# Farama-Foundation/Gymnasium-Robotics

Hardware: NVIDIA H100
Metric: env-steps/s (higher is better)
Workload: dtype f32

## Files before the change

### gymnasium_robotics_b200/csrc/sim_core.cuh

```cuda
#pragma once
#include "dmodel.h"

#if defined(__CUDACC__) || defined(B200_HOST_WARP)
#define B200_WARP_CODE 1
#endif
#ifdef __CUDACC__
#define HD static __device__ __forceinline__
#define HDN static __device__ __noinline__
#define STAGE static __device__ __noinline__
#define ASSUME_SHARED_PTR(p) __builtin_assume(__isShared(p))
#define ASSUME_SHARED(c) do { __builtin_assume(__isShared((c).s)); __builtin_assume(__isShared((c).mw)); __builtin_assume(__isShared((c).h)); } while (0)
#define WARP_W 32
#define SYNC() __syncwarp()
#define ALIGN() __syncthreads()
#define ALIGN_OR(p) __syncthreads_or(p)
#elif defined(B200_HOST_WARP)
#define HD static inline
#define HDN static
#define STAGE static
#define ASSUME_SHARED(c) do { } while (0)
#define ASSUME_SHARED_PTR(p) do { } while (0)
#define WARP_W 32
#define SYNC() __syncwarp()
#define ALIGN() __syncwarp()
// ... 1221 lines not shown
        else if (t2 == B200_GEOM_SPHERE) collide_plane_sphere(c, g1, g2, margin, o);
        else collide_plane_capsule(c, g1, g2, margin, o);
      } else if (t1 == B200_GEOM_BOX) collide_box_box(c, g1, g2, margin, o, bs);
      else if (t2 == B200_GEOM_BOX) collide_round_box(c, g1, g2, margin, o);
      else if (HF) collide_round_round(c, g1, g2, margin, o);
      float inc = margin - GF(pair_gap)[p];
      int k2 = 0;
      for (int k = 0; k < o.cnt; k++) if (o.dist[k] < inc) { if (k2 != k) { o.dist[k2] = o.dist[k]; for (int a = 0; a < 3; a++) { o.pos[k2][a] = o.pos[k][a]; o.nrm[k2][a] = o.nrm[k][a]; } } k2++; }
      o.cnt = k2;
    }
    int ocnt = o.cnt;
    int gtotal, gslot = wexscan(ocnt > 0 ? 1 : 0, c.lane, &gtotal);
    int basec = cnt[CNT_NCON], baseg = cnt[CNT_NGRP];
    int gid = baseg + gslot;
    if (ocnt > 0 && gid >= h->ngrp_max - DM_NWELD_MAX) ocnt = 0;
    int total, slot = wexscan(ocnt, c.lane, &total);
    SYNC();
    int kept = 0;
    for (int k = 0; k < ocnt; k++) {
      int id = basec + slot + k;
      if (id >= h->ncon_max) break;
      float* cr = SF(con) + id * CON_WORDS;
      cr[0] = o.pos[k][0]; cr[1] = o.pos[k][1]; cr[2] = o.pos[k][2];
      cr[3] = o.nrm[k][0]; cr[4] = o.nrm[k][1]; cr[5] = o.nrm[k][2];
      cr[6] = o.dist[k];
      ((int*)cr)[7] = p;
      ((int*)cr)[C_DIMGRP] = gid << 8;
      kept++;
    }
    if (ocnt > 0) {
      int* gi = (int*)(SF(group) + gid * GRP_WORDS);
      int ba = MI(geom_body)[PAIR_I(pair_geom1)[p]], bb = PAIR_I(pair_geom2)[p] < 0 ? 0 : MI(geom_body)[PAIR_I(pair_geom2)[p]];
      dmask_t ma = DM(body_ancdof, ba), mb = DM(body_ancdof, bb);
      const int bodies = GI(geom_mjb)[PAIR_I(pair_geom1)[p]] | ((PAIR_I(pair_geom2)[p] < 0 ? 0 : GI(geom_mjb)[PAIR_I(pair_geom2)[p]]) << 8);
      ((uint32_t*)gi)[G_RANGE] = (uint32_t)(basec + slot) | (uint32_t)kept << 8 | (uint32_t)bodies << 16;
      grp_set_masks(gi, ma ^ mb, mb);
    }
    if (c.lane == 0) {
      int nn = basec + total; if (nn > h->ncon_max) { nn = h->ncon_max; cnt[CNT_OVERFLOW] |= 2; }
      int ng = baseg + gtotal; if (ng > h->ngrp_max - DM_NWELD_MAX) { ng = h->ngrp_max - DM_NWELD_MAX; cnt[CNT_OVERFLOW] |= 4; }
      cnt[CNT_NCON] = nn; cnt[CNT_NGRP] = ng;
    }
    SYNC();
  }
  LANES(id, cnt[CNT_NCON]) {
    float* cr = SF(con) + id * CON_WORDS;
    const float pos[3] = {cr[0], cr[1], cr[2]}, dist = cr[6];
    float fr9[9] = {cr[3], cr[4], cr[5], 0, 0, 0, 0, 0, 0};
    const int p = ((const int*)cr)[7], gid8 = ((const int*)cr)[C_DIMGRP];
    make_frame(fr9);
    float r[3] = {pos[0] - h->ref[0], pos[1] - h->ref[1], pos[2] - h->ref[2]};
    for (int a = 0; a < 3; a++) { float* w = cr + C_W + 6 * a; cross3(w, r, fr9 + 3 * a); w[3] = fr9[3 * a]; w[4] = fr9[3 * a + 1]; w[5] = fr9[3 * a + 2]; }
    const float* fr = GF(pair_friction) + 3 * p;
    int dim = GI(pair_condim)[p];
    float mu0 = fr[0];
    cr[C_MU] = mu0; cr[C_MU + 1] = fr[1];
#ifdef B200_KITCHEN
    cr[C_MU + 2] = fr[2];
#endif
    float incl = PAIR_F(pair_margin)[p] - GF(pair_gap)[p];
    float solimp[5] = {GF(pair_solimp)[5 * p], GF(pair_solimp)[5 * p + 1], GF(pair_solimp)[5 * p + 2], GF(pair_solimp)[5 * p + 3], GF(pair_solimp)[5 * p + 4]};
    float solref[2] = {GF(pair_solref)[2 * p], GF(pair_solref)[2 * p + 1]};
    float imp = impedance(solimp, dist, incl);
    float K, Bc;
    ref_kb(c, solref, solimp[1], &K, &Bc);
    float tran = GF(pair_invweight)[2 * p];
    float R;
    if (dim == 1) R = fmaxf((1 - imp) / imp * tran, B200_MINVAL);
    else {
      float R0 = fmaxf((1 - imp) / imp * (tran + mu0 * mu0 * tran), B200_MINVAL);
      float mu = mu0 * rsqrtf(h->impratio);
      R = fmaxf(2 * mu * mu * R0, B200_MINVAL);
    }
    cr[C_D] = 1.0f / R;
    cr[C_U] = K * imp * (dist - incl); cr[C_U + 1] = 0; cr[C_U + 2] = 0; cr[C_U + 3] = 0;
#ifdef B200_KITCHEN
    cr[C_U + 4] = 0; cr[C_U + 5] = 0;
#endif
    cr[C_JV] = Bc;
    ((int*)cr)[C_DIMGRP] = dim | gid8;
    if (HF && h->nsensor > 0) {
      float* cx = SF(conx) + id * CX_WORDS;
      cx[CX_POS] = pos[0]; cx[CX_POS + 1] = pos[1]; cx[CX_POS + 2] = pos[2];
      ((int*)cx)[CX_PAIR] = p;
    }
  }
  SYNC();
}

#ifdef B200_KITCHEN
HD void con_w(const float* cr, int k, float* w) {
  if (k < 3) { const float* s = cr + C_W + 6 * k; w[0] = s[0]; w[1] = s[1]; w[2] = s[2]; w[3] = s[3]; w[4] = s[4]; w[5] = s[5]; }
  else { const float* s = cr + C_W + 6 * (k - 3) + 3; w[0] = s[0]; w[1] = s[1]; w[2] = s[2]; w[3] = w[4] = w[5] = 0; }
}
HD float con_mu(const float* cr, int k) { return k < 3 ? cr[C_MU] : (k == 3 ? cr[C_MU + 1] : cr[C_MU + 2]); }
#else
HD void con_w(const float* cr, int k, float* w) {
  if (k < 3) { const float* s = cr + C_W + 6 * k; w[0] = s[0]; w[1] = s[1]; w[2] = s[2]; w[3] = s[3]; w[4] = s[4]; w[5] = s[5]; }
  else { w[0] = cr[C_W + 3]; w[1] = cr[C_W + 4]; w[2] = cr[C_W + 5]; w[3] = w[4] = w[5] = 0; }
}
HD float con_mu(const float* cr, int k) { return k < 3 ? cr[C_MU] : cr[C_MU + 1]; }
#endif
HD int con_dim(const float* cr) { return ((const int*)cr)[C_DIMGRP] & 0xff; }
HD int con_grp(const float* cr) { return (((const int*)cr)[C_DIMGRP] >> 8) & 0xff; }
HD uint32_t con_act(const float* cr) { return ((const uint32_t*)cr)[C_DIMGRP] >> 16; }

template <bool HF>
STAGE void make_constraint(const Ctx c) {
  ASSUME_SHARED(c);
  const DMHead* h = c.h;
  int* cnt = SI(counters);
  if (c.lane == 0) { cnt[CNT_NDR] = 0; cnt[CNT_NWELD] = 0; }
  SYNC();
  for (int e = 0; e < h->neq; e++) {
    if (!MI(eq_active)[e] || MI(eq_type)[e] != B200_EQ_WELD) continue;
    const int nw = cnt[CNT_NWELD], gid = cnt[CNT_NGRP];
    float* wr = SF(weld) + nw * WELD_WORDS;
    const float* data = MF(eq_data) + 11 * e;
    int s1 = MI(eq_obj1)[e], s2 = MI(eq_obj2)[e], b1 = 0, b2 = 0;
    float p1[3] = {0, 0, 0}, p2[3] = {0, 0, 0}, q1[4] = {1, 0, 0, 0}, q2[4] = {1, 0, 0, 0}, t[3];
    if (s1 >= 0) { b1 = MI(site_body)[s1]; qmul(q1, SF(xquat) + 4 * b1, MF(site_quat) + 4 * s1); qrot(t, SF(xquat) + 4 * b1, MF(site_pos) + 3 * s1); for (int k = 0; k < 3; k++) p1[k] = SF(xpos)[3 * b1 + k] + t[k]; }
    if (s2 >= 0) { b2 = MI(site_body)[s2]; qmul(q2, SF(xquat) + 4 * b2, MF(site_quat) + 4 * s2); qrot(t, SF(xquat) + 4 * b2, MF(site_pos) + 3 * s2); for (int k = 0; k < 3; k++) p2[k] = SF(xpos)[3 * b2 + k] + t[k]; }
    qrot(t, q1, data + 3); for (int k = 0; k < 3; k++) p1[k] += t[k];
    qrot(t, q2, data + 0); for (int k = 0; k < 3; k++) p2[k] += t[k];
    const float ts = data[10];
    float quat[4], quat1[4] = {q2[0], -q2[1], -q2[2], -q2[3]}, quat2[4];
    qmul(quat, q1, data + 6);
    qmul(quat2, quat1, quat);
    const bool use1 = b1 > 0 && DM(body_ancdof, b1) != 0;
    float r[3];
    for (int k = 0; k < 3; k++) r[k] = (use1 ? p1[k] : p2[k]) - h->ref[k];
    float K, Bc;
    ref_kb(c, MF(eq_solref) + 2 * e, MF(eq_solimp)[5 * e + 1], &K, &Bc);
    LANES(k, 6) {
      float* w = wr + W_W + 6 * k;
      float cp;
      if (k < 3) {
        float e3[3] = {k == 0 ? 1.f : 0.f, k == 1 ? 1.f : 0.f, k == 2 ? 1.f : 0.f};
        cross3(w, r, e3); w[3] = e3[0]; w[4] = e3[1]; w[5] = e3[2];
        cp = k == 0 ? p1[0] - p2[0] : (k == 1 ? p1[1] - p2[1] : p1[2] - p2[2]);
      } else {
        const int kk = k - 3;
        for (int a = 0; a < 3; a++) {
          float qa[4] = {0, a == 0 ? 1.f : 0.f, a == 1 ? 1.f : 0.f, a == 2 ? 1.f : 0.f}, t1[4], t2[4];
          qmul(t1, quat1, qa); qmul(t2, t1, quat);
          w[a] = 0.5f * ts * (kk == 0 ? t2[1] : (kk == 1 ? t2[2] : t2[3])); w[3 + a] = 0;
        }
        cp = ts * (kk == 0 ? quat2[1] : (kk == 1 ? quat2[2] : quat2[3]));
      }
      float imp = impedance(MF(eq_solimp) + 5 * e, cp, 0.f);
      float R = fmaxf((1 - imp) / imp * MF(eq_invweight)[2 * e + (k < 3 ? 0 : 1)], B200_MINVAL);
      wr[W_D + k] = 1.0f / R; wr[W_JAR + k] = K * imp * cp;
    }
    if (c.lane == 0) {
      wr[W_B] = Bc;
      ((int*)wr)[W_GRP] = gid;
      int* gi = (int*)(SF(group) + gid * GRP_WORDS);
      dmask_t ma = DM(body_ancdof, b2), mb = DM(body_ancdof, b1);
      gi[G_RANGE] = 0;
      grp_set_masks(gi, ma ^ mb, mb);
    }
    SYNC();
    if (c.lane == 0) { cnt[CNT_NGRP] = gid + 1; cnt[CNT_NWELD] = nw + 1; }
    SYNC();
  }
  for (int base = 0; base < h->njnt; base += WARP_W) {
    int j = base + c.lane;
    int nrow = 0; float dist0 = 0, dist1 = 0, sgn0 = 0, sgn1 = 0;
    if (j < h->njnt && MI(jnt_limited)[j] && MI(jnt_type)[j] != B200_JNT_FREE) {
      float q = SF(qpos)[MI(jnt_qposadr)[j]], margin = MF(jnt_margin)[j];
      float dl = q - MF(jnt_range)[2 * j], du = MF(jnt_range)[2 * j + 1] - q;
      if (dl < margin) { dist0 = dl; sgn0 = 1.f; nrow = 1; }
      if (du < margin) { if (nrow) { dist1 = du; sgn1 = -1.f; } else { dist0 = du; sgn0 = -1.f; } nrow++; }
    }
    int total, slot = wexscan(nrow, c.lane, &total);
    int basec = cnt[CNT_NDR];
    SYNC();
#pragma unroll
    for (int k = 0; k < 2; k++) {
      int id = basec + slot + k;
      if (k >= nrow || id >= h->ndr_max) continue;
      const float distk = k ? dist1 : dist0, sgnk = k ? sgn1 : sgn0;
      float* dr = SF(dofrow) + id * DR_WORDS;
      int* di = (int*)dr;
      int d = MI(jnt_dofadr)[j];
      float margin = MF(jnt_margin)[j];
      float solimp[5] = {GF(jnt_solimp)[5 * j], GF(jnt_solimp)[5 * j + 1], GF(jnt_solimp)[5 * j + 2], GF(jnt_solimp)[5 * j + 3], GF(jnt_solimp)[5 * j + 4]};
      float solref[2] = {GF(jnt_solref)[2 * j], GF(jnt_solref)[2 * j + 1]};
      float imp = impedance(solimp, distk, margin);
      float K, Bc;
      ref_kb(c, solref, solimp[1], &K, &Bc);
      float R = fmaxf((1 - imp) / imp * MF(dof_invweight0)[d], B200_MINVAL);
      di[DR_DOF] = d; dr[DR_COEF] = sgnk; di[DR_DOF2] = -1; dr[DR_COEF2] = 0;
      dr[DR_D] = 1.0f / R; dr[DR_JAR] = K * imp * (distk - margin); dr[DR_JV] = Bc;
    }
    if (c.lane == 0) { int nn = basec + total; if (nn > h->ndr_max) { nn = h->ndr_max; cnt[CNT_OVERFLOW] |= 8; } cnt[CNT_NDR] = nn; }
    SYNC();
  }
  if (HF) for (int base = 0; base < h->nten; base += WARP_W) {
    int t = base + c.lane;
    int nrow = 0; float dist0 = 0, dist1 = 0, sgn0 = 0, sgn1 = 0;
    if (t < h->nten) {
      float len = MF(ten_coef)[2 * t] * SF(qpos)[MI(ten_qadr)[2 * t]];
      if (MI(ten_dof)[2 * t + 1] >= 0) len += MF(ten_coef)[2 * t + 1] * SF(qpos)[MI(ten_qadr)[2 * t + 1]];
      float margin = MF(ten_margin)[t];
      float dl = len - MF(ten_range)[2 * t], du = MF(ten_range)[2 * t + 1] - len;
      if (dl < margin) { dist0 = dl; sgn0 = 1.f; nrow = 1; }
      if (du < margin) { if (nrow) { dist1 = du; sgn1 = -1.f; } else { dist0 = du; sgn0 = -1.f; } nrow++; }
    }
    int total, slot = wexscan(nrow, c.lane, &total);
    int basec = cnt[CNT_NDR];
    SYNC();
#pragma unroll
    for (int k = 0; k < 2; k++) {
      int id = basec + slot + k;
      if (k >= nrow || id >= h->ndr_max) continue;
      const float distk = k ? dist1 : dist0, sgnk = k ? sgn1 : sgn0;
      float* dr = SF(dofrow) + id * DR_WORDS;
      int* di = (int*)dr;
      float margin = MF(ten_margin)[t];
      float solimp[5] = {GF(ten_solimp)[5 * t], GF(ten_solimp)[5 * t + 1], GF(ten_solimp)[5 * t + 2], GF(ten_solimp)[5 * t + 3], GF(ten_solimp)[5 * t + 4]};
      float solref[2] = {GF(ten_solref)[2 * t], GF(ten_solref)[2 * t + 1]};
      float imp = impedance(solimp, distk, margin);
      float K, Bc;
      ref_kb(c, solref, solimp[1], &K, &Bc);
      float R = fmaxf((1 - imp) / imp * GF(ten_invweight)[t], B200_MINVAL);
      di[DR_DOF] = MI(ten_dof)[2 * t]; dr[DR_COEF] = sgnk * MF(ten_coef)[2 * t];
      di[DR_DOF2] = MI(ten_dof)[2 * t + 1]; dr[DR_COEF2] = sgnk * MF(ten_coef)[2 * t + 1];
      dr[DR_D] = 1.0f / R; dr[DR_JAR] = K * imp * (distk - margin); dr[DR_JV] = Bc;
    }
    if (c.lane == 0) { int nn = basec + total; if (nn > h->ndr_max) { nn = h->ndr_max; cnt[CNT_OVERFLOW] |= 8; } cnt[CNT_NDR] = nn; }
    SYNC();
  }
#ifdef B200_KITCHEN
  if (c.lane == 0) {
    for (int e = 0; e < h->neq; e++) {
      if (!MI(eq_active)[e] || MI(eq_type)[e] != B200_EQ_JOINT) continue;
      int id = cnt[CNT_NDR];
      if (id >= h->ndr_max) { cnt[CNT_OVERFLOW] |= 8; break; }
      const float* data = MF(eq_data) + 11 * e;
      int j1 = MI(eq_obj1)[e], j2 = MI(eq_obj2)[e];
      float pos = SF(qpos)[MI(jnt_qposadr)[j1]] - MF(jnt_qpos0)[j1], deriv = 0.f;
      if (j2 >= 0) {
        float dif = SF(qpos)[MI(jnt_qposadr)[j2]] - MF(jnt_qpos0)[j2];
        pos -= data[0] + dif * (data[1] + dif * (data[2] + dif * (data[3] + dif * data[4])));
        deriv = data[1] + dif * (2 * data[2] + dif * (3 * data[3] + dif * 4 * data[4]));
      } else pos -= data[0];
      float* dr = SF(dofrow) + id * DR_WORDS;
      int* di = (int*)dr;
      float imp = impedance(MF(eq_solimp) + 5 * e, pos, 0.f);
      float K, Bc;
      ref_kb(c, MF(eq_solref) + 2 * e, MF(eq_solimp)[5 * e + 1], &K, &Bc);
      float R = fmaxf((1 - imp) / imp * MF(eq_invweight)[2 * e], B200_MINVAL);
      di[DR_DOF] = MI(jnt_dofadr)[j1]; dr[DR_COEF] = 1.f;
      di[DR_DOF2] = j2 >= 0 ? MI(jnt_dofadr)[j2] : -1; dr[DR_COEF2] = -deriv;
      dr[DR_D] = -1.0f / R; dr[DR_JAR] = K * imp * pos; dr[DR_JV] = Bc;
      cnt[CNT_NDR] = id + 1;
    }
  }
  SYNC();
#endif
  if (HF) { LANES(d, h->nfric) SF(fric)[d] = 0.f; SYNC(); }
}

HD uint32_t contact_base_forces(const float* cr, int dim, const float (&U)[C_NB], float* F) {
  float D = cr[C_D], un = U[0];
#pragma unroll
  for (int k = 0; k < C_NB; k++) F[k] = 0;
  if (dim == 1) { F[0] = un < 0 ? -D * un : 0.f; return un < 0 ? 1u : 0u; }
  uint32_t act = 0;
#pragma unroll
  for (int k = 1; k < C_NB; k++) {
    if (k >= dim) continue;
    float mu = con_mu(cr, k), uk = U[k];
    float xp = un + mu * uk, xm = un - mu * uk;
    float fp = xp < 0 ? -D * xp : 0.f, fm = xm < 0 ? -D * xm : 0.f;
    act |= (xp < 0 ? 1u : 0u) << (2 * k - 2) | (xm < 0 ? 1u : 0u) << (2 * k - 1);
    F[0] += fp + fm;
    F[k] = mu * (fp - fm);
  }
  return act;
}
HD void contact_base_forces(const float* cr, int dim, float* F) {
  float U[C_NB];
#pragma unroll
  for (int k = 0; k < C_NB; k++) U[k] = cr[C_U + k];
  contact_base_forces(cr, dim, U, F);
}
HD void contact_park_forces(float* cr, const float (&U)[C_NB]) {
  int* dg = (int*)cr + C_DIMGRP;
  float F[C_NB];
  const uint32_t act = contact_base_forces(cr, *dg & 0xff, U, F);
#pragma unroll
  for (int k = 0; k < C_NB; k++) cr[C_JV + k] = F[k];
  *dg = (int)(((uint32_t)*dg & 0xffffu) | act << 16);
}

template <bool HF>
STAGE void rows_from_vec(const Ctx c, const float* vec) {
  ASSUME_SHARED(c);
  ASSUME_SHARED_PTR(vec);
  const int* cnt = SI(counters);
  int ngrp = cnt[CNT_NGRP];
  LANES(idx, ngrp * 6) {
    int g = idx / 6, a = idx - 6 * g;
    float* gr = SF(group) + g * GRP_WORDS;
    dmask_t S = grp_mask(gr), sg = grp_sign(gr);
    float acc = 0;
    while (S) { int j = ffs_pop(S); float t = SF(cdof)[6 * j + a] * vec[j]; acc += DBIT(sg, j) ? t : -t; }
    gr[G_V + a] = acc;
  }
  SYNC();
  LANES(i, cnt[CNT_NCON]) {
    float* cr = SF(con) + i * CON_WORDS;
    int dim = con_dim(cr), nbase = dim == 1 ? 1 : dim;
    const float* dV = SF(group) + con_grp(cr) * GRP_WORDS + G_V;
    for (int k = 0; k < nbase; k++) {
      float w[6];
      con_w(cr, k, w);
      cr[C_JV + k] = dot6(w, dV);
    }
  }
  LANES(i, cnt[CNT_NWELD] * 6) {
    float* wr = SF(weld) + (i / 6) * WELD_WORDS;
    int k = i % 6;
    const float* dV = SF(group) + ((const int*)wr)[W_GRP] * GRP_WORDS + G_V;
    wr[W_JV + k] = dot6(wr + W_W + 6 * k, dV);
  }
  LANES(i, cnt[CNT_NDR]) {
    float* dr = SF(dofrow) + i * DR_WORDS;
    const int* di = (const int*)dr;
    float val = dr[DR_COEF] * vec[di[DR_DOF]];
    if (di[DR_DOF2] >= 0) val += dr[DR_COEF2] * vec[di[DR_DOF2]];
    dr[DR_JV] = val;
  }
  if (HF) LANES(d, c.h->nfric) SF(fric)[c.h->nfric + d] = vec[d];
  SYNC();
}

template <bool HF>
STAGE void rows_begin(const Ctx c, const float* qvel, const float* qacc) {
  ASSUME_SHARED(c);
  ASSUME_SHARED_PTR(qvel); ASSUME_SHARED_PTR(qacc);
  const int* cnt = SI(counters);
  int ngrp = cnt[CNT_NGRP];
  float* dA = SF(H);
  LANES(idx, ngrp * 6) {
    int g = idx / 6, a = idx - 6 * g;
    float* gr = SF(group) + g * GRP_WORDS;
    dmask_t S = grp_mask(gr), sg = grp_sign(gr);
    float acc = 0, acc2 = 0;
    while (S) {
      int j = ffs_pop(S);
      float cd = SF(cdof)[6 * j + a], t = cd * qvel[j], t2 = cd * qacc[j];
      bool pos = DBIT(sg, j);
      acc += pos ? t : -t; acc2 += pos ? t2 : -t2;
    }
    gr[G_V + a] = acc; dA[idx] = acc2;
  }
  SYNC();
  LANES(i, cnt[CNT_NCON]) {
    float* cr = SF(con) + i * CON_WORDS;
    int dim = con_dim(cr), nbase = dim == 1 ? 1 : dim;
    const float* gr = SF(group) + con_grp(cr) * GRP_WORDS;
    const float* gA = dA + 6 * con_grp(cr);
    float Bc = cr[C_JV];
    float U[C_NB];
#pragma unroll
    for (int k = 0; k < C_NB; k++) {
      U[k] = 0.f;
      if (k >= nbase) continue;
      float w[6];
      con_w(cr, k, w);
      float u = cr[C_U + k];
      u += Bc * dot6(w, gr + G_V);
      u += dot6(w, gA);
      cr[C_U + k] = u;
      U[k] = u;
    }
    contact_park_forces(cr, U);
  }
  LANES(i, cnt[CNT_NWELD] * 6) {
    float* wr = SF(weld) + (i / 6) * WELD_WORDS;
    int k = i % 6;
    const int g = ((const int*)wr)[W_GRP];
    const float* gr = SF(group) + g * GRP_WORDS;
    float u = wr[W_JAR + k];
    u += wr[W_B] * dot6(wr + W_W + 6 * k, gr + G_V);
    u += dot6(wr + W_W + 6 * k, dA + 6 * g);
    wr[W_JAR + k] = u;
  }
  LANES(i, cnt[CNT_NDR]) {
    float* dr = SF(dofrow) + i * DR_WORDS;
    const int* di = (const int*)dr;
    float v1 = dr[DR_COEF] * qvel[di[DR_DOF]], v2 = dr[DR_COEF] * qacc[di[DR_DOF]];
    if (di[DR_DOF2] >= 0) { v1 += dr[DR_COEF2] * qvel[di[DR_DOF2]]; v2 += dr[DR_COEF2] * qacc[di[DR_DOF2]]; }
    float u = dr[DR_JAR];
    u += dr[DR_JV] * v1;
    u += v2;
    dr[DR_JAR] = u;
  }
  if (HF) LANES(d, c.h->nfric) {
    float* fr = SF(fric);
    float u = fr[d];
    u += MF(dof_fricB)[d] * qvel[d];
    u += qacc[d];
    fr[d] = u;
  }
  SYNC();
}

template <bool HF>
HD void pass_F(const Ctx c, float* out) {
  ASSUME_SHARED(c);
  const DMHead* h = c.h;
  const int* cnt = SI(counters);
  int ngrp = cnt[CNT_NGRP], nweld = cnt[CNT_NWELD], ndr = cnt[CNT_NDR];
  LANES(idx, ngrp * 6) {
    int g = idx / 6, a = idx - 6 * g;
    float* gr = SF(group) + g * GRP_WORDS;
    float acc = 0;
    for (int i = grp_start(gr), i1 = i + grp_count(gr); i < i1; i++) {
      const float* cr = SF(con) + i * CON_WORDS;
      int dim = con_dim(cr);
      const float* F = cr + C_JV;
      acc += F[0] * cr[C_W + a];
      if (dim > 1) acc += F[1] * cr[C_W + 6 + a] + F[2] * cr[C_W + 12 + a];
      if (dim > 3 && a < 3) acc += F[3] * cr[C_W + 3 + a];
#ifdef B200_KITCHEN
      if (dim > 4 && a < 3) acc += F[4] * cr[C_W + 6 + 3 + a] + F[5] * cr[C_W + 12 + 3 + a];
#endif
    }
    for (int i = 0; i < nweld; i++) {
      const float* wr = SF(weld) + i * WELD_WORDS;
      if (((const int*)wr)[W_GRP] != g) continue;
      for (int k = 0; k < 6; k++) acc -= wr[W_D + k] * wr[W_JAR + k] * wr[W_W + 6 * k + a];
    }
    gr[G_V + a] = acc;
  }
  SYNC();
  LANES(j, h->nv) {
    float q = 0;
    const float* cd = SF(cdof) + 6 * j;
    for (int g = 0; g < ngrp; g++) {
      const float* gr = SF(group) + g * GRP_WORDS;
      if (!DBIT(grp_mask(gr), j)) continue;
      float d = dot6(cd, gr + G_V);
      q += DBIT(grp_sign(gr), j) ? d : -d;
    }
    for (int i = 0; i < ndr; i++) {
      const float* dr = SF(dofrow) + i * DR_WORDS;
      const int* di = (const int*)dr;
      float x = dr[DR_JAR];
#ifdef B200_KITCHEN
      float f = (dr[DR_D] < 0 || x < 0) ? -fabsf(dr[DR_D]) * x : 0.f;
#else
      float f = x < 0 ? -dr[DR_D] * x : 0.f;
#endif
      if (di[DR_DOF] == j) q += dr[DR_COEF] * f;
      if (di[DR_DOF2] == j) q += dr[DR_COEF2] * f;
    }
    if (HF && h->nfric) {
      float fl = MF(dof_frictionloss)[j];
      q += fminf(fmaxf(-MF(dof_fricD)[j] * SF(fric)[j], -fl), fl);
    }
    out[j] = q;
  }
  SYNC();
}

STAGE void mulM(const Ctx c, const float* v, float* out) {
  ASSUME_SHARED(c);
  ASSUME_SHARED_PTR(v); ASSUME_SHARED_PTR(out);
  int nv = c.h->nv;
  const float* M = SF(M);
  LANES(i, nv) {
    float a = 0;
    const int row = i * (i + 1) / 2;
    for (int j = 0; j <= i; j++) a += M[row + j] * v[j];
    for (int j = i + 1, idx = row + 2 * i + 1; j < nv; idx += ++j) a += M[idx] * v[j];
    out[i] = a;
  }
  SYNC();
}

template <bool HF>
STAGE void build_H(const Ctx c) {
  ASSUME_SHARED(c);
  const DMHead* h = c.h;
  const int* cnt = SI(counters);
  int nv = h->nv, nM = nv * (nv + 1) / 2, nweld = cnt[CNT_NWELD], ngrp = cnt[CNT_NGRP], ndr = cnt[CNT_NDR];
  float* H = SF(H);
  LANES(i, nM) H[i] = SF(M)[i];
  float* Kc = H + nM;
  const int kcap = (h->s_grad - h->s_H - nM) / 21;
  for (int g0 = 0; g0 < ngrp; g0 += kcap) {
    const int g1 = ngrp - g0 < kcap ? ngrp : g0 + kcap;
    LANES(e, 21) {
      int r = 0; while ((r + 1) * (r + 2) / 2 <= e) r++;
      const int s = e - r * (r + 1) / 2;
      for (int g = g0; g < g1; g++) {
        float* K = Kc + 21 * (g - g0);
        const float* gr = SF(group) + g * GRP_WORDS;
        float acc = 0;
        for (int i = grp_start(gr), i1 = i + grp_count(gr); i < i1; i++) {
          const float* cr = SF(con) + i * CON_WORDS;
          const int dim = con_dim(cr);
          const uint32_t act = con_act(cr);
          float D = cr[C_D];
          float wnr = cr[C_W + r], wns = cr[C_W + s];
          if (dim == 1) { if (act & 1u) acc += D * wnr * wns; continue; }
          float Wnn = 0;
          for (int k = 1; k < dim; k++) {
            float ap = (act >> (2 * k - 2)) & 1u ? 1.f : 0.f, am = (act >> (2 * k - 1)) & 1u ? 1.f : 0.f;
            if (ap + am == 0.f) continue;
            float mu = con_mu(cr, k);
            float wkr, wks;
            if (k < 3) { wkr = cr[C_W + 6 * k + r]; wks = cr[C_W + 6 * k + s]; }
#ifdef B200_KITCHEN
            else { wkr = r < 3 ? cr[C_W + 6 * (k - 3) + 3 + r] : 0.f; wks = s < 3 ? cr[C_W + 6 * (k - 3) + 3 + s] : 0.f; }
#else
            else { wkr = r < 3 ? cr[C_W + 3 + r] : 0.f; wks = s < 3 ? cr[C_W + 3 + s] : 0.f; }
#endif
            Wnn += ap + am;
            float Wnk = mu * (ap - am), Wkk = mu * mu * (ap + am);
            acc += D * (Wnk * (wnr * wks + wkr * wns) + Wkk * wkr * wks);
          }
          acc += D * Wnn * wnr * wns;
        }
        for (int i = 0; i < nweld; i++) {
          const float* wr = SF(weld) + i * WELD_WORDS;
          if (((const int*)wr)[W_GRP] != g) continue;
          for (int k = 0; k < 6; k++) acc += wr[W_D + k] * wr[W_W + 6 * k + r] * wr[W_W + 6 * k + s];
        }
        K[e] = acc;
      }
    }
    SYNC();
    LANES(i, nv) {
      const float* cd = SF(cdof) + 6 * i;
      const int row = i * (i + 1) / 2;
      for (int g = g0; g < g1; g++) {
        const float* gr = SF(group) + g * GRP_WORDS;
        const dmask_t S = grp_mask(gr), mb = grp_sign(gr);
        if (!DBIT(S, i)) continue;
        const float* K = Kc + 21 * (g - g0);
        float y[6];
#pragma unroll
        for (int r = 0; r < 6; r++) {
          float a = 0;
#pragma unroll
          for (int s2 = 0; s2 < 6; s2++) a += K[pidx(r, s2)] * cd[s2];
          y[r] = a;
        }
        float si = DBIT(mb, i) ? 1.f : -1.f;
        dmask_t m2 = S & (((dmask_t)2 << i) - (dmask_t)1);
        while (m2) {
          int j = ffs_pop(m2);
          float sj = DBIT(mb, j) ? 1.f : -1.f;
          H[row + j] += si * sj * dot6(SF(cdof) + 6 * j, y);
        }
      }
    }
    SYNC();
  }
  SYNC();
  if (HF) {
    LANES(d, h->nfric) {
      float D = MF(dof_fricD)[d], x = SF(fric)[d];
      if (D > 0 && fabsf(x) * D < MF(dof_frictionloss)[d]) H[d * (d + 1) / 2 + d] += D;
    }
    SYNC();
  }
  if (HF) {
    LANES(j, nv) {
      float diag = 0.f;
      for (int i = 0; i < ndr; i++) {
        const float* dr = SF(dofrow) + i * DR_WORDS;
        const int* di = (const int*)dr;
#ifdef B200_KITCHEN
        if (!(dr[DR_JAR] < 0 || dr[DR_D] < 0)) continue;
        const float Dr = fabsf(dr[DR_D]);
#else
        if (!(dr[DR_JAR] < 0)) continue;
        const float& Dr = dr[DR_D];
#endif
        int d1 = di[DR_DOF], d2 = di[DR_DOF2];
        if (d1 == j) diag += Dr * dr[DR_COEF] * dr[DR_COEF];
        if (d2 == j) diag += Dr * dr[DR_COEF2] * dr[DR_COEF2];
        if (d2 >= 0 && (d1 > d2 ? d1 : d2) == j) H[j * (j + 1) / 2 + (d1 > d2 ? d2 : d1)] += Dr * dr[DR_COEF] * dr[DR_COEF2];
      }
      H[j * (j + 1) / 2 + j] += diag;
    }
  } else if (c.lane == 0) {
    for (int i = 0; i < ndr; i++) {
      const float* dr = SF(dofrow) + i * DR_WORDS;
      const int* di = (const int*)dr;
      if (!(dr[DR_JAR] < 0)) continue;
      int d1 = di[DR_DOF], d2 = di[DR_DOF2];
      H[pidx(d1, d1)] += dr[DR_D] * dr[DR_COEF] * dr[DR_COEF];
      if (d2 >= 0) { H[pidx(d2, d2)] += dr[DR_D] * dr[DR_COEF2] * dr[DR_COEF2]; H[pidx(d1, d2)] += dr[DR_D] * dr[DR_COEF] * dr[DR_COEF2]; }
    }
  }
  SYNC();
}

STAGE void cholesky(const Ctx c, float* H) {
  ASSUME_SHARED(c);
  int n = c.h->nv;
  for (int k = 0; k < n; k++) {
    float hkk = H[k * (k + 1) / 2 + k];
    float d = sqrtf(fmaxf(hkk, 1e-30f)), inv = 1.0f / d;
    SYNC();
    LANES(i, n) { if (i == k) H[i * (i + 1) / 2 + k] = d; else if (i > k) H[i * (i + 1) / 2 + k] *= inv; }
    SYNC();
    LANES(i, n) {
      if (i <= k) continue;
      int row = i * (i + 1) / 2;
      float lik = H[row + k];
      for (int j = k + 1; j <= i; j++) H[row + j] -= lik * H[j * (j + 1) / 2 + k];
    }
    SYNC();
  }
}
STAGE void chol_solve(const Ctx c, const float* L, float* x) {
  ASSUME_SHARED(c);
  int n = c.h->nv;
  for (int k = 0; k < n; k++) {
    if (c.lane == (k % WARP_W)) x[k] = x[k] / L[k * (k + 1) / 2 + k];
    SYNC();
    float xk = x[k];
    LANES(i, n) if (i > k) x[i] -= L[i * (i + 1) / 2 + k] * xk;
    SYNC();
  }
  for (int k = n - 1; k >= 0; k--) {
    if (c.lane == (k % WARP_W)) x[k] = x[k] / L[k * (k + 1) / 2 + k];
    SYNC();
    float xk = x[k];
    LANES(i, k) x[i] -= L[k * (k + 1) / 2 + i] * xk;
    SYNC();
  }
}

#ifdef B200_WARP_CODE
template <int NVP>
static __device__ __noinline__ void spd_solve(const Ctx c, const float* A, const float* dadd, float hh, float* x, float* scratchH) {
  ASSUME_SHARED(c);
  __builtin_assume(__isShared(A)); __builtin_assume(__isShared(x)); if (dadd) __builtin_assume(__isShared(dadd));
  __builtin_assume(__isShared(scratchH));
  constexpr int NA = NVP > 32 ? 32 : NVP, KB = NVP > 32 ? NVP - 32 : 0, KS = KB > 0 ? KB : 1;
  const int nv = c.h->nv, i = c.lane;
  const unsigned FULL = 0xffffffffu;
  float h[NA];
  const int rowi = i * (i + 1) / 2;
  const bool live = i < nv;
#pragma unroll
  for (int j = 0; j < NA; j++) {
    const bool in = live && j < nv;
    int idx = (j <= i) ? rowi + j : j * (j + 1) / 2 + i;
    idx = in ? idx : 0;
    float v = A[idx];
    v = in ? v : ((i == j) ? 1.f : 0.f);
    h[j] = v;
  }
  float cb[KS], S[KS][KS], bb[KS];
#pragma unroll
  for (int r = 0; r < KB; r++) {
    const int row = 32 + r, ro = row * (row + 1) / 2;
    const bool in = row < nv;
    cb[r] = (in && live) ? A[ro + i] : 0.f;
#pragma unroll
    for (int q = 0; q < KB; q++) {
      const int col = 32 + q;
      const bool in2 = in && col < nv;
      float v = A[in2 ? (q <= r ? ro + col : col * (col + 1) / 2 + row) : 0];
      S[r][q] = in2 ? v : (r == q ? 1.f : 0.f);
    }
    bb[r] = in ? x[row] : 0.f;
  }
  if (dadd != nullptr) {
    float dd = hh * dadd[live ? i : 0];
#pragma unroll
    for (int j = 0; j < NA; j++) h[j] += (live && i == j) ? dd : 0.f;
#pragma unroll
    for (int r = 0; r < KB; r++) S[r][r] += (32 + r < nv) ? hh * dadd[32 + r < nv ? 32 + r : 0] : 0.f;
  }
  float b = 0.f;
  if (live) b = x[i];
  float dinv = 1.f;
  constexpr int NA4 = (NA + 3) & ~3;
  float* colbuf = scratchH;
  __syncwarp();
#pragma unroll
  for (int k = 0; k < NA; k++) {
    float hkk = __shfl_sync(FULL, h[k], k);
    float inv = rsqrtf(fmaxf(hkk, 1e-30f));
    float lik = (i > k) ? h[k] * inv : 0.f;
    dinv = (i == k) ? inv : dinv;
    h[k] = (i > k) ? lik : h[k];
    if (k + 1 < NA) {
      float* col = colbuf + (k & 1) * NA4;
      if (i < NA4) col[i] = lik;
      __syncwarp();
      const float4* c4 = (const float4*)col;
#pragma unroll
      for (int q = (k + 1) / 4; q < NA4 / 4; q++) {
        const float4 v = c4[q];
        if (4 * q + 0 > k && 4 * q + 0 < NA) h[4 * q + 0] = fmaf(-lik, v.x, h[4 * q + 0]);
        if (4 * q + 1 > k && 4 * q + 1 < NA) h[4 * q + 1] = fmaf(-lik, v.y, h[4 * q + 1]);
        if (4 * q + 2 > k && 4 * q + 2 < NA) h[4 * q + 2] = fmaf(-lik, v.z, h[4 * q + 2]);
        if (4 * q + 3 > k && 4 * q + 3 < NA) h[4 * q + 3] = fmaf(-lik, v.w, h[4 * q + 3]);
      }
    }
    float lr[KS];
#pragma unroll
    for (int r = 0; r < KB; r++) {
      lr[r] = __shfl_sync(FULL, cb[r] * inv, k);
      cb[r] = (i == k) ? lr[r] : fmaf(-lr[r], lik, cb[r]);
    }
#pragma unroll
    for (int r = 0; r < KB; r++)
#pragma unroll
      for (int q = 0; q < KB; q++) S[r][q] = fmaf(-lr[r], lr[q], S[r][q]);
  }
  float sinv[KS];
#pragma unroll
  for (int k = 0; k < KB; k++) {
    float inv = rsqrtf(fmaxf(S[k][k], 1e-30f));
    sinv[k] = inv;
#pragma unroll
    for (int r = k + 1; r < KB; r++) S[r][k] *= inv;
#pragma unroll
    for (int r = k + 1; r < KB; r++)
#pragma unroll
      for (int q = k + 1; q <= r; q++) S[r][q] = fmaf(-S[r][k], S[q][k], S[r][q]);
  }
#pragma unroll
  for (int k = 0; k < NA; k++) {
    float yk = __shfl_sync(FULL, b * dinv, k);
    float bn = fmaf(-h[k], yk, b);
    b = (i > k) ? bn : ((i == k) ? yk : b);
  }
#pragma unroll
  for (int r = 0; r < KB; r++) bb[r] -= wsum(cb[r] * b);
#pragma unroll
  for (int k = 0; k < KB; k++) {
    bb[k] *= sinv[k];
#pragma unroll
    for (int r = k + 1; r < KB; r++) bb[r] = fmaf(-S[r][k], bb[k], bb[r]);
  }
#pragma unroll
  for (int k = KB - 1; k >= 0; k--) {
    bb[k] *= sinv[k];
#pragma unroll
    for (int r = 0; r < k; r++) bb[r] = fmaf(-S[k][r], bb[k], bb[r]);
  }
#pragma unroll
  for (int r = 0; r < KB; r++) b = fmaf(-cb[r], bb[r], b);
  float sacc = 0.f, z = 0.f;
#pragma unroll
  for (int k = NA - 1; k >= 0; k--) {
    float zk = __shfl_sync(FULL, (b - dinv * sacc) * dinv, k);
    float sn = fmaf(h[k], zk, sacc);
    sacc = (i < k) ? sn : sacc;
    z = (i == k) ? zk : z;
  }
  __syncwarp();
  if (i < nv && i < NA) x[i] = z;
#pragma unroll
  for (int r = 0; r < KB; r++) if (i == r && 32 + r < nv) x[32 + r] = bb[r];
  __syncwarp();
}
#else
template <int NVP>
static inline void spd_solve(const Ctx& c, const float* A, const float* dadd, float hh, float* x, float* scratchH) {
  int nv = c.h->nv, nM = nv * (nv + 1) / 2;
  for (int i = 0; i < nM; i++) scratchH[i] = A[i];
  if (dadd) for (int i = 0; i < nv; i++) scratchH[i * (i + 1) / 2 + i] += hh * dadd[i];
  cholesky(c, scratchH);
  chol_solve(c, scratchH, x);
}
#endif

struct LsStep { float alpha, improve; };
#ifndef B200_KITCHEN
struct LsVal { float cost, d1, d2; };

HD float pyramid_edge(float xn, float mu, float xk) {
#ifdef __CUDACC__
  return fmaf(mu, xk, xn);
#else
  return xn + mu * xk;
#endif
}

template <bool HF, int NS>
HD LsVal ls_eval(const Ctx c, const float (&ex)[NS], const float (&ev)[NS], const float (&eD)[NS], int nedge, float alpha, float g1,
                 float g2) {
  float cost = 0, d1 = 0, d2 = 0;
#pragma unroll
  for (int j = 0; j < NS; j++) {
    if (WARP_W * j >= nedge) break;
    float x0 = ex[j], v = ev[j], D = eD[j];
    float x = fmaf(alpha, v, x0), Da = fabsf(D);
    if (D < 0 || (x < 0 && D > 0)) { float dx = Da * x; cost = fmaf(0.5f * dx, x, cost); d1 = fmaf(dx, v, d1); d2 = fmaf(Da * v, v, d2); }
  }
  if (HF) LANES(d, c.h->nfric) {
    float D = MF(dof_fricD)[d];
    if (D > 0) {
      float fl = MF(dof_frictionloss)[d], v = SF(fric)[c.h->nfric + d], x = SF(fric)[d] + alpha * v, Rf = fl / D;
      if (x <= -Rf) { cost += fl * (-0.5f * Rf - x); d1 -= fl * v; }
      else if (x >= Rf) { cost += fl * (-0.5f * Rf + x); d1 += fl * v; }
      else { cost += 0.5f * D * x * x; d1 += D * x * v; d2 += D * v * v; }
    }
  }
  LsVal r;
  r.cost = wsum(cost) + alpha * g1 + alpha * alpha * g2;
  r.d1 = wsum(d1) + g1 + 2 * alpha * g2;
  r.d2 = wsum(d2) + 2 * g2;
  return r;
}

template <bool HF, int LSE>
HD LsStep linesearch(const Ctx c, float g1, float g2, float gtol, int maxit) {
  ASSUME_SHARED(c);
  constexpr int NS = LSE * 32 / WARP_W;
  const DMHead* h = c.h;
  const int* cnt = SI(counters);
  const int epc = h->edges_per_con, ncon = cnt[CNT_NCON], nweld6 = cnt[CNT_NWELD] * 6, ndr = cnt[CNT_NDR];
  const int nce = epc * ncon, nwe = nce + nweld6, nedge = nwe + ndr;
  float ex[NS], ev[NS], eD[NS];
  const int qs = WARP_W / epc, rs = WARP_W % epc;
  int q = c.lane / epc, r = c.lane % epc;
#pragma unroll
  for (int j = 0; j < NS; j++) {
    const int e = c.lane + WARP_W * j;
    float x0 = 0.f, v = 0.f, D = 0.f;
    if (j > 0) { q += qs; r += rs; if (r >= epc) { r -= epc; q++; } }
    if (WARP_W * j < nedge) {
      if (e < nce) {
        const float* cr = SF(con) + q * CON_WORDS;
        const int k = r, dim = con_dim(cr);
        const float un = cr[C_U], vn = cr[C_JV];
        if (dim == 1) {
          if (k == 0) { x0 = un; v = vn; D = cr[C_D]; }
        } else if (k < 2 * (dim - 1)) {
          const int b = 1 + (k >> 1);
          const float mu = con_mu(cr, b), su = (k & 1) ? -cr[C_U + b] : cr[C_U + b], sv = (k & 1) ? -cr[C_JV + b] : cr[C_JV + b];
          x0 = pyramid_edge(un, mu, su); v = pyramid_edge(vn, mu, sv);
          D = cr[C_D];
        }
      } else if (e < nwe) {
        const int i = e - nce;
        const float* wr = SF(weld) + (i / 6) * WELD_WORDS;
        x0 = wr[W_JAR + i % 6]; v = wr[W_JV + i % 6]; D = -wr[W_D + i % 6];
      } else if (e < nedge) {
        const float* dr = SF(dofrow) + (e - nwe) * DR_WORDS;
        x0 = dr[DR_JAR]; v = dr[DR_JV]; D = dr[DR_D];
      }
    }
    ex[j] = x0; ev[j] = v; eD[j] = D;
  }
  const LsVal p0 = ls_eval<HF>(c, ex, ev, eD, nedge, 0.f, g1, g2);
  if (p0.d1 >= 0 || p0.d2 <= 0) return LsStep{0.f, 0.f};
  gtol = fmaxf(gtol, 1e-5f * fabsf(p0.d1));
  float lo = 0, hi = -1, alpha = -p0.d1 / p0.d2, best = 0, bestcost = p0.cost;
  for (int it = 0; it < maxit; it++) {
    const LsVal p = ls_eval<HF>(c, ex, ev, eD, nedge, alpha, g1, g2);
    if (p.cost <= bestcost) { bestcost = p.cost; best = alpha; }
    if (fabsf(p.d1) < gtol) break;
    if (p.d1 < 0) lo = alpha; else hi = alpha;
    float next = alpha - p.d1 / p.d2;
    if (hi > 0 && (next <= lo || next >= hi)) next = 0.5f * (lo + hi);
    if (next == alpha) break;
    alpha = next;
  }
  return LsStep{best, p0.cost - bestcost};
}

#else
template <bool HF>
STAGE int ls_edges(const Ctx c) {
  ASSUME_SHARED(c);
  const DMHead* h = c.h;
  const int* cnt = SI(counters);
  const int epc = h->edges_per_con, ncon = cnt[CNT_NCON], nweld6 = cnt[CNT_NWELD] * 6, ndr = cnt[CNT_NDR];
  float* E = SF(H);
  LANES(i, ncon) {
    const float* cr = SF(con) + i * CON_WORDS;
    float* e = E + 3 * epc * i;
    int dim = con_dim(cr);
    float D = cr[C_D], un = cr[C_U], vn = cr[C_JV];
    int ne = 0;
    if (dim == 1) { e[0] = un; e[1] = vn; e[2] = D; ne = 1; }
    else for (int k = 1; k < dim; k++) {
      float mu = con_mu(cr, k), uk = mu * cr[C_U + k], vk = mu * cr[C_JV + k];
      e[3 * ne] = un + uk; e[3 * ne + 1] = vn + vk; e[3 * ne + 2] = D; ne++;
      e[3 * ne] = un - uk; e[3 * ne + 1] = vn - vk; e[3 * ne + 2] = D; ne++;
    }
    for (; ne < epc; ne++) e[3 * ne + 2] = 0.f;
  }
  float* W = E + 3 * epc * ncon;
  LANES(i, nweld6) {
    const float* wr = SF(weld) + (i / 6) * WELD_WORDS;
    int k = i % 6;
    W[3 * i] = wr[W_JAR + k]; W[3 * i + 1] = wr[W_JV + k]; W[3 * i + 2] = -wr[W_D + k];
  }
  float* R = W + 3 * nweld6;
  LANES(i, ndr) {
    const float* dr = SF(dofrow) + i * DR_WORDS;
    R[3 * i] = dr[DR_JAR]; R[3 * i + 1] = dr[DR_JV]; R[3 * i + 2] = dr[DR_D];
  }
  SYNC();
  return epc * ncon + nweld6 + ndr;
}

template <bool HF>
STAGE void ls_eval(const Ctx c, int nedge, float alpha, float g1, float g2, float* out) {
  ASSUME_SHARED(c);
  float cost = 0, d1 = 0, d2 = 0;
  const float* E = SF(H);
  LANES(i, nedge) {
    float x0 = E[3 * i], v = E[3 * i + 1], D = E[3 * i + 2];
    float x = fmaf(alpha, v, x0), Da = fabsf(D);
    if (D < 0 || (x < 0 && D > 0)) { float dx = Da * x; cost = fmaf(0.5f * dx, x, cost); d1 = fmaf(dx, v, d1); d2 = fmaf(Da * v, v, d2); }
  }
  if (HF) LANES(d, c.h->nfric) {
    float D = MF(dof_fricD)[d];
    if (D > 0) {
      float fl = MF(dof_frictionloss)[d], v = SF(fric)[c.h->nfric + d], x = SF(fric)[d] + alpha * v, Rf = fl / D;
      if (x <= -Rf) { cost += fl * (-0.5f * Rf - x); d1 -= fl * v; }
      else if (x >= Rf) { cost += fl * (-0.5f * Rf + x); d1 += fl * v; }
      else { cost += 0.5f * D * x * x; d1 += D * x * v; d2 += D * v * v; }
    }
  }
  out[0] = wsum(cost) + alpha * g1 + alpha * alpha * g2;
  out[1] = wsum(d1) + g1 + 2 * alpha * g2;
  out[2] = wsum(d2) + 2 * g2;
}

template <bool HF, int LSE>
STAGE LsStep linesearch(const Ctx c, float g1, float g2, float gtol, int maxit) {
  ASSUME_SHARED(c);
  float p0[3], p[3];
  const int nedge = ls_edges<HF>(c);
  ls_eval<HF>(c, nedge, 0.f, g1, g2, p0);
  if (p0[1] >= 0 || p0[2] <= 0) return LsStep{0.f, 0.f};
  gtol = fmaxf(gtol, 1e-5f * fabsf(p0[1]));
  float lo = 0, hi = -1, alpha = -p0[1] / p0[2], best = 0, bestcost = p0[0];
  for (int it = 0; it < maxit; it++) {
    ls_eval<HF>(c, nedge, alpha, g1, g2, p);
    if (p[0] <= bestcost) { bestcost = p[0]; best = alpha; }
    if (fabsf(p[1]) < gtol) break;
    if (p[1] < 0) lo = alpha; else hi = alpha;
    float next = alpha - p[1] / p[2];
    if (hi > 0 && (next <= lo || next >= hi)) next = 0.5f * (lo + hi);
    if (next == alpha) break;
    alpha = next;
  }
  return LsStep{best, p0[0] - bestcost};
}

#endif


template <bool HF>
HD int newton_check(const Ctx c, int iter, float improvement) {
  ASSUME_SHARED(c);
  const DMHead* h = c.h;
  int nv = h->nv;
  float *Ma = SF(Ma), *grad = SF(grad), *fs = SF(fsmooth), *fcon = SF(fcon);
  float scale = 1.0f / (h->meaninertia * (float)(nv > 1 ? nv : 1));
  float tol = fmaxf(h->tolerance, 1e-6f);
  TIC();
  pass_F<HF>(c, fcon);
  TOC(TM_CK_PASSF);
  float g2sum = 0, f2sum = 0;
  LANES(i, nv) {
    float g = Ma[i] - fs[i] - fcon[i], f = fabsf(Ma[i]) + fabsf(fs[i]) + fabsf(fcon[i]);
    grad[i] = g; g2sum += g * g; f2sum += f * f;
  }
  SYNC();
  float gnorm = sqrtf(wsum(g2sum)), fnorm = sqrtf(wsum(f2sum));
  if (gnorm < 2e-6f * fnorm) return 1;
  if (iter > 0 && (scale * improvement < tol || scale * gnorm < tol)) return 1;
  if (iter >= h->iterations || iter >= 12) return 1;
  return 0;
}

template <bool HF>
STAGE int newton_begin(const Ctx c) {
  ASSUME_SHARED(c);
  mulM(c, SF(qacc), SF(Ma));
  rows_begin<HF>(c, SF(qvel), SF(qacc));
  CHECK_TIC();
  const int done = newton_check<HF>(c, 0, 0.f);
  CHECK_TOC(TM_NBEGIN);
  return done;
}

template <int NVP>
STAGE void newton_direction(const Ctx c) {
  ASSUME_SHARED(c);
  int nv = c.h->nv;
  LANES(i, nv) SF(search)[i] = -SF(grad)[i];
  SYNC();
  spd_solve<NVP>(c, SF(H), nullptr, 0.f, SF(search), SF(H));
}

template <bool HF, int LSE>
STAGE int newton_move(const Ctx c, int iter) {
  ASSUME_SHARED(c);
  const DMHead* h = c.h;
  int nv = h->nv;
  int* cnt = SI(counters);
  float *a = SF(qacc), *Ma = SF(Ma), *Mv = SF(Mv), *search = SF(search), *fs = SF(fsmooth);
  float scale = 1.0f / (h->meaninertia * (float)(nv > 1 ? nv : 1));
  TIC();
  mulM(c, search, Mv);
  TOC(TM_MV_MULM);
  rows_from_vec<HF>(c, search);
  TOC(TM_MV_ROWS);
  float q1 = 0, q2 = 0, sn = 0;
  LANES(i, nv) { q1 += search[i] * (Ma[i] - fs[i]); q2 += 0.5f * search[i] * Mv[i]; sn += search[i] * search[i]; }
  q1 = wsum(q1); q2 = wsum(q2); sn = sqrtf(wsum(sn));
  if (sn < 1e-20f) return 2;
  float gtol = h->tolerance * h->ls_tolerance * sn / scale;
  TOC(TM_MV_ROWS);
  const LsStep ls = linesearch<HF, LSE>(c, q1, q2, gtol, h->ls_iterations < 20 ? h->ls_iterations : 20);
  const float alpha = ls.alpha;
  TOC(TM_MV_LS);
  if (alpha == 0.f) return 2;
  LANES(i, nv) { a[i] += alpha * search[i]; Ma[i] += alpha * Mv[i]; }
  LANES(i, cnt[CNT_NCON]) {
    float* cr = SF(con) + i * CON_WORDS;
    float U[C_NB];
#pragma unroll
    for (int k = 0; k < C_NB; k++) { U[k] = cr[C_U + k] + alpha * cr[C_JV + k]; cr[C_U + k] = U[k]; }
    contact_park_forces(cr, U);
  }
  LANES(i, cnt[CNT_NWELD] * 6) { float* wr = SF(weld) + (i / 6) * WELD_WORDS; wr[W_JAR + i % 6] += alpha * wr[W_JV + i % 6]; }
  LANES(i, cnt[CNT_NDR]) { float* dr = SF(dofrow) + i * DR_WORDS; dr[DR_JAR] += alpha * dr[DR_JV]; }
  if (HF) LANES(d, h->nfric) SF(fric)[d] += alpha * SF(fric)[h->nfric + d];
  SYNC();
  if (c.lane == 0) cnt[CNT_ITERS] += 1;
  TOC(TM_MV_UPD);
  CHECK_TIC();
  const int done = newton_check<HF>(c, iter + 1, ls.improve);
  CHECK_TOC(TM_NMOVE);
  return done;
}

template <int NVP>
STAGE void euler_solve(const Ctx c) {
  ASSUME_SHARED(c);
  const DMHead* h = c.h;
  float* x = SF(search);
  LANES(i, h->nv) x[i] = SF(fsmooth)[i] + SF(fcon)[i];
  SYNC();
  spd_solve<NVP>(c, SF(M), MF(dof_damping), h->timestep, x, SF(H));
}

template <int NVP, bool REBUILD = false>
HD void forward(const Ctx c, bool active) {
  constexpr bool HF = NVP >= 30;
  constexpr bool CX = NVP == 22 || NVP >= 30;
  constexpr int kLsE = DM_LS_E(NVP);
  TIC();
  ALIGN(); TOC(TM_BARRIER);
  if (active) kinematics(stage_ctx<REBUILD>(c));
  TOC(TM_KIN); if (HF) ALIGN(); TOC(TM_BARRIER);
  if (active) { com_quantities(stage_ctx<REBUILD>(c)); mass_matrix(stage_ctx<REBUILD>(c)); }
  TOC(TM_COM_M); ALIGN(); TOC(TM_BARRIER);
  if (active) collision<HF, CX>(stage_ctx<REBUILD>(c));
  TOC(TM_COLL); if (!REBUILD) ALIGN(); TOC(TM_BARRIER);
  if (active) make_constraint<HF>(stage_ctx<REBUILD>(c));
  TOC(TM_CONSTR); if (HF) ALIGN(); TOC(TM_BARRIER);
  if (active) smooth_forces(stage_ctx<REBUILD>(c));
  TOC(TM_SMOOTH); if (HF) ALIGN(); TOC(TM_BARRIER);
  int done = 1;
  if (active) done = newton_begin<HF>(stage_ctx<REBUILD>(c));
  TOC(TM_NBEGIN);
  for (int iter = 0;; iter++) {
    bool more = ALIGN_OR(!done);
    TOC(TM_BARRIER);
    if (!more) break;
    if (!done) build_H<HF>(stage_ctx<REBUILD>(c));
    TOC(TM_BUILDH); if (HF) ALIGN(); TOC(TM_BARRIER);
    if (!done) newton_direction<NVP>(stage_ctx<REBUILD>(c));
    TOC(TM_NDIR); if (!REBUILD) ALIGN(); TOC(TM_BARRIER);
    if (!done) done = newton_move<HF, kLsE>(stage_ctx<REBUILD>(c), iter);
    TOC(TM_NMOVE);
  }
}

STAGE void integrate_pos(const Ctx c, float* qpos, const float* qvel, float hh) {
  ASSUME_SHARED(c);
  ASSUME_SHARED_PTR(qpos); ASSUME_SHARED_PTR(qvel);
  const DMHead* h = c.h;
  LANES(j, h->njnt) {
    int a = MI(jnt_qposadr)[j], d = MI(jnt_dofadr)[j];
    if (MI(jnt_type)[j] == B200_JNT_FREE) {
      for (int k = 0; k < 3; k++) qpos[a + k] += hh * qvel[d + k];
      float w[3] = {qvel[d + 3], qvel[d + 4], qvel[d + 5]};
      float n = sqrtf(dot3(w, w));
      float q[4] = {qpos[a + 3], qpos[a + 4], qpos[a + 5], qpos[a + 6]};
      if (n > 0) {
        float ang = 0.5f * n * hh, sn = sinf(ang), cs = cosf(ang), inv = 1.0f / n;
        float dq[4] = {cs, w[0] * inv * sn, w[1] * inv * sn, w[2] * inv * sn}, nq[4];
        qmul(nq, q, dq);
        q[0] = nq[0]; q[1] = nq[1]; q[2] = nq[2]; q[3] = nq[3];
      }
      qnormalize(q);
      qpos[a + 3] = q[0]; qpos[a + 4] = q[1]; qpos[a + 5] = q[2]; qpos[a + 6] = q[3];
    } else qpos[a] += hh * qvel[d];
  }
  SYNC();
}

template <int NVP>
STAGE void euler_step(const Ctx c) {
  ASSUME_SHARED(c);
  const DMHead* h = c.h;
  int nv = h->nv;
  float hh = h->timestep;
  float* x = SF(search);
  if (h->any_damping) {
    euler_solve<NVP>(c);
  } else {
    LANES(i, nv) x[i] = SF(qacc)[i];
    SYNC();
  }
  LANES(i, nv) SF(qvel)[i] += hh * x[i];
  SYNC();
  integrate_pos(c, SF(qpos), SF(qvel), hh);
}

template <int NVP, bool REBUILD = false>
HD void rk4_substep(const Ctx c, bool active) {
  const DMHead* h = c.h;
  const int nv = h->nv, nq = h->nq;
  const float hh = h->timestep;
  const float A[3] = {0.5f, 0.5f, 1.0f}, B[4] = {1.0f / 6, 1.0f / 3, 1.0f / 3, 1.0f / 6};
  if (active) {
    LANES(i, nq) SF(rk_q0)[i] = SF(qpos)[i];
    LANES(i, nv) { SF(rk_v0)[i] = SF(qvel)[i]; SF(rk_dx)[i] = B[0] * SF(qvel)[i]; SF(rk_df)[i] = B[0] * SF(qacc)[i]; }
    SYNC();
  }
  for (int st = 1; st < 4; st++) {
    if (active) {
      float a = A[st - 1] * hh;
      LANES(i, nq) SF(qpos)[i] = SF(rk_q0)[i];
      SYNC();
      integrate_pos(c, SF(qpos), SF(qvel), a);
      LANES(i, nv) SF(qvel)[i] = SF(rk_v0)[i] + a * SF(qacc)[i];
      SYNC();
    }
    forward<NVP, REBUILD>(c, active);
    if (active) {
      LANES(i, nv) { SF(rk_dx)[i] += B[st] * SF(qvel)[i]; SF(rk_df)[i] += B[st] * SF(qacc)[i]; }
      SYNC();
    }
  }
  if (active) {
    LANES(i, nq) SF(qpos)[i] = SF(rk_q0)[i];
    LANES(i, nv) SF(qvel)[i] = SF(rk_v0)[i] + hh * SF(rk_df)[i];
    SYNC();
    integrate_pos(c, SF(qpos), SF(rk_dx), hh);
  }
}
```

Before: 1.136 million.

## Shrink solver code size with unroll-1 loops, inline mulM, approx rsqrt

Adds `#pragma unroll 1` to many warp-strided loops in the row, Newton and update stages. It makes mulM an inline helper instead of a noinline stage and splits the gradient-norm computation into its own noinline function. The first line-search evaluation is folded into the main loop so ls_eval is instantiated once. Cholesky rsqrt now uses inline rsqrt.approx.ftz PTX. The aim is smaller code, less instruction-cache pressure and fewer register spills, at the cost of less ILP in the small loops and flush-to-zero rsqrt semantics.

Result: faster. 1.160 million (median of 6 runs) (+2.0%).

```diff
diff --git a/gymnasium_robotics_b200/csrc/sim_core.cuh b/gymnasium_robotics_b200/csrc/sim_core.cuh
--- a/gymnasium_robotics_b200/csrc/sim_core.cuh
+++ b/gymnasium_robotics_b200/csrc/sim_core.cuh
@@ -1547,6 +1547,7 @@
   ASSUME_SHARED_PTR(vec);
   const int* cnt = SI(counters);
   int ngrp = cnt[CNT_NGRP];
+#pragma unroll 1
   LANES(idx, ngrp * 6) {
     int g = idx / 6, a = idx - 6 * g;
     float* gr = SF(group) + g * GRP_WORDS;
@@ -1556,22 +1557,26 @@
     gr[G_V + a] = acc;
   }
   SYNC();
+#pragma unroll 1
   LANES(i, cnt[CNT_NCON]) {
     float* cr = SF(con) + i * CON_WORDS;
     int dim = con_dim(cr), nbase = dim == 1 ? 1 : dim;
     const float* dV = SF(group) + con_grp(cr) * GRP_WORDS + G_V;
+#pragma unroll 1
     for (int k = 0; k < nbase; k++) {
       float w[6];
       con_w(cr, k, w);
       cr[C_JV + k] = dot6(w, dV);
     }
   }
+#pragma unroll 1
   LANES(i, cnt[CNT_NWELD] * 6) {
     float* wr = SF(weld) + (i / 6) * WELD_WORDS;
     int k = i % 6;
     const float* dV = SF(group) + ((const int*)wr)[W_GRP] * GRP_WORDS + G_V;
     wr[W_JV + k] = dot6(wr + W_W + 6 * k, dV);
   }
+#pragma unroll 1
   LANES(i, cnt[CNT_NDR]) {
     float* dr = SF(dofrow) + i * DR_WORDS;
     const int* di = (const int*)dr;
@@ -1714,15 +1719,17 @@
   SYNC();
 }
 
-STAGE void mulM(const Ctx c, const float* v, float* out) {
-  ASSUME_SHARED(c);
-  ASSUME_SHARED_PTR(v); ASSUME_SHARED_PTR(out);
+HD void mulM(const Ctx c, const float* v, float* out) {
+  ASSUME_SHARED(c);
   int nv = c.h->nv;
   const float* M = SF(M);
+#pragma unroll 1
   LANES(i, nv) {
     float a = 0;
     const int row = i * (i + 1) / 2;
+#pragma unroll 1
     for (int j = 0; j <= i; j++) a += M[row + j] * v[j];
+#pragma unroll 1
     for (int j = i + 1, idx = row + 2 * i + 1; j < nv; idx += ++j) a += M[idx] * v[j];
     out[i] = a;
   }
@@ -1888,6 +1895,15 @@
 }
 
 #ifdef B200_WARP_CODE
+HD float rsqrt_normal(float x) {
+#ifdef __CUDACC__
+  float r;
+  asm("rsqrt.approx.ftz.f32 %0, %1;" : "=f"(r) : "f"(x));
+  return r;
+#else
+  return rsqrtf(x);
+#endif
+}
 template <int NVP>
 static __device__ __noinline__ void spd_solve(const Ctx c, const float* A, const float* dadd, float hh, float* x, float* scratchH) {
   ASSUME_SHARED(c);
@@ -1939,10 +1955,10 @@
 #pragma unroll
   for (int k = 0; k < NA; k++) {
     float hkk = __shfl_sync(FULL, h[k], k);
-    float inv = rsqrtf(fmaxf(hkk, 1e-30f));
-    float lik = (i > k) ? h[k] * inv : 0.f;
+    float inv = rsqrt_normal(fmaxf(hkk, 1e-30f));
     dinv = (i == k) ? inv : dinv;
-    h[k] = (i > k) ? lik : h[k];
+    h[k] *= (i > k) ? inv : 1.f;
+    const float lik = (i > k) ? h[k] : 0.f;
     if (k + 1 < NA) {
       float* col = colbuf + (k & 1) * NA4;
       if (i < NA4) col[i] = lik;
@@ -1971,7 +1987,7 @@
   float sinv[KS];
 #pragma unroll
   for (int k = 0; k < KB; k++) {
-    float inv = rsqrtf(fmaxf(S[k][k], 1e-30f));
+    float inv = rsqrt_normal(fmaxf(S[k][k], 1e-30f));
     sinv[k] = inv;
 #pragma unroll
     for (int r = k + 1; r < KB; r++) S[r][k] *= inv;
@@ -2106,12 +2122,16 @@
     }
     ex[j] = x0; ev[j] = v; eD[j] = D;
   }
-  const LsVal p0 = ls_eval<HF>(c, ex, ev, eD, nedge, 0.f, g1, g2);
-  if (p0.d1 >= 0 || p0.d2 <= 0) return LsStep{0.f, 0.f};
-  gtol = fmaxf(gtol, 1e-5f * fabsf(p0.d1));
-  float lo = 0, hi = -1, alpha = -p0.d1 / p0.d2, best = 0, bestcost = p0.cost;
-  for (int it = 0; it < maxit; it++) {
+  float lo = 0, hi = -1, alpha = 0.f, best = 0, bestcost = 0, cost0 = 0;
+#pragma unroll 1
+  for (int it = -1; it < maxit; it++) {
     const LsVal p = ls_eval<HF>(c, ex, ev, eD, nedge, alpha, g1, g2);
+    if (it < 0) {
+      if (p.d1 >= 0 || p.d2 <= 0) return LsStep{0.f, 0.f};
+      gtol = fmaxf(gtol, 1e-5f * fabsf(p.d1));
+      alpha = -p.d1 / p.d2; bestcost = cost0 = p.cost;
+      continue;
+    }
     if (p.cost <= bestcost) { bestcost = p.cost; best = alpha; }
     if (fabsf(p.d1) < gtol) break;
     if (p.d1 < 0) lo = alpha; else hi = alpha;
@@ -2120,7 +2140,7 @@
     if (next == alpha) break;
     alpha = next;
   }
-  return LsStep{best, p0.cost - bestcost};
+  return LsStep{best, cost0 - bestcost};
 }
 
 #else
@@ -2209,26 +2229,34 @@
 #endif
 
 
+struct GradNorms { float g, f; };
 template <bool HF>
-HD int newton_check(const Ctx c, int iter, float improvement) {
-  ASSUME_SHARED(c);
-  const DMHead* h = c.h;
-  int nv = h->nv;
+HDN GradNorms newton_grad(const Ctx c) {
+  ASSUME_SHARED(c);
+  int nv = c.h->nv;
   float *Ma = SF(Ma), *grad = SF(grad), *fs = SF(fsmooth), *fcon = SF(fcon);
-  float scale = 1.0f / (h->meaninertia * (float)(nv > 1 ? nv : 1));
-  float tol = fmaxf(h->tolerance, 1e-6f);
   TIC();
   pass_F<HF>(c, fcon);
   TOC(TM_CK_PASSF);
   float g2sum = 0, f2sum = 0;
+#pragma unroll 1
   LANES(i, nv) {
     float g = Ma[i] - fs[i] - fcon[i], f = fabsf(Ma[i]) + fabsf(fs[i]) + fabsf(fcon[i]);
     grad[i] = g; g2sum += g * g; f2sum += f * f;
   }
   SYNC();
-  float gnorm = sqrtf(wsum(g2sum)), fnorm = sqrtf(wsum(f2sum));
-  if (gnorm < 2e-6f * fnorm) return 1;
-  if (iter > 0 && (scale * improvement < tol || scale * gnorm < tol)) return 1;
+  return GradNorms{sqrtf(wsum(g2sum)), sqrtf(wsum(f2sum))};
+}
+
+template <bool HF>
+HD int newton_check(const Ctx c, int iter, float improvement) {
+  const DMHead* h = c.h;
+  int nv = h->nv;
+  float scale = 1.0f / (h->meaninertia * (float)(nv > 1 ? nv : 1));
+  float tol = fmaxf(h->tolerance, 1e-6f);
+  const GradNorms n = newton_grad<HF>(c);
+  if (n.g < 2e-6f * n.f) return 1;
+  if (iter > 0 && (scale * improvement < tol || scale * n.g < tol)) return 1;
   if (iter >= h->iterations || iter >= 12) return 1;
   return 0;
 }
@@ -2267,6 +2295,7 @@
   rows_from_vec<HF>(c, search);
   TOC(TM_MV_ROWS);
   float q1 = 0, q2 = 0, sn = 0;
+#pragma unroll 1
   LANES(i, nv) { q1 += search[i] * (Ma[i] - fs[i]); q2 += 0.5f * search[i] * Mv[i]; sn += search[i] * search[i]; }
   q1 = wsum(q1); q2 = wsum(q2); sn = sqrtf(wsum(sn));
   if (sn < 1e-20f) return 2;
@@ -2276,7 +2305,9 @@
   const float alpha = ls.alpha;
   TOC(TM_MV_LS);
   if (alpha == 0.f) return 2;
+#pragma unroll 1
   LANES(i, nv) { a[i] += alpha * search[i]; Ma[i] += alpha * Mv[i]; }
+#pragma unroll 1
   LANES(i, cnt[CNT_NCON]) {
     float* cr = SF(con) + i * CON_WORDS;
     float U[C_NB];
@@ -2284,7 +2315,9 @@
     for (int k = 0; k < C_NB; k++) { U[k] = cr[C_U + k] + alpha * cr[C_JV + k]; cr[C_U + k] = U[k]; }
     contact_park_forces(cr, U);
   }
+#pragma unroll 1
   LANES(i, cnt[CNT_NWELD] * 6) { float* wr = SF(weld) + (i / 6) * WELD_WORDS; wr[W_JAR + i % 6] += alpha * wr[W_JV + i % 6]; }
+#pragma unroll 1
   LANES(i, cnt[CNT_NDR]) { float* dr = SF(dofrow) + i * DR_WORDS; dr[DR_JAR] += alpha * dr[DR_JV]; }
   if (HF) LANES(d, h->nfric) SF(fric)[d] += alpha * SF(fric)[h->nfric + d];
   SYNC();
```
